# lawfuyang/ToyRenderer

Measured on AMD Instinct MI355X. Metric: Gmeshlets/s culled (whole node), 100M meshlets, higher is better.
Workload: dtype f32

## Files before the change

toyrenderer_amd/csrc/cull_math.hip.h:

```cpp
#pragma once

#include <hip/hip_runtime.h>

#include "ShaderInterop.h"

namespace cm
{

struct F3 { float x, y, z; };

__device__ __forceinline__ float fma_(float a, float b, float c) { return __builtin_fmaf(a, b, c); }
__device__ __forceinline__ float min_(float a, float b) { return __builtin_fminf(a, b); }
__device__ __forceinline__ float max_(float a, float b) { return __builtin_fmaxf(a, b); }
#ifdef TR_EXPERIMENT_FAST_MATH
__device__ __forceinline__ float sqrt_(float a) { return __builtin_amdgcn_sqrtf(a); }
__device__ __forceinline__ float div_(float a, float b) { return a * __builtin_amdgcn_rcpf(b); }
#else
__device__ __forceinline__ float sqrt_(float a) { return __builtin_sqrtf(a); }
__device__ __forceinline__ float div_(float a, float b) { return a / b; }
#endif
__device__ __forceinline__ float clamp_(float x, float lo, float hi) { return min_(max_(x, lo), hi); }

typedef unsigned long long lmask;
__device__ __forceinline__ lmask mLt(float a, float b) { lmask m; asm("v_cmp_lt_f32_e64 %0, %1, %2" : "=s"(m) : "v"(a), "v"(b)); return m; }
// ... 222 lines not shown

__device__ __forceinline__ bool occlusionResolve(const OccSample& o, uint32_t row0, uint32_t row1)
{
    float d00 = texelLo(row0), d10 = texelLo(row1);
    float d01 = o.pair ? texelHi(row0) : d00, d11 = o.pair ? texelHi(row1) : d10;
    float depth = min_(min_(min_(d00, d01), d10), d11);
    return o.accept | (o.depthSphere >= depth);
}

struct HzbQuad
{
    const _Float16* base;
    uint32_t total;
    uint32_t offset[16];
};
__device__ __forceinline__ uint32_t quadIndex(uint32_t offset, uint32_t blockRowStride , uint32_t X, uint32_t Y)
{
    return offset + (__umul24(Y >> 3, blockRowStride) + ((Y << 3) & 56u)) + __umul24(X >> 3, 56u) + X;
}

struct OccQuad
{
    lmask accept;
    lmask slow;
    float depthSphere;
    uint32_t iq;
};

__device__ __forceinline__ bool occlusionVisible(F3 c, float r, float nearPlane, float P00, float P11, const Hzb& h)
{
    if ((c.z - nearPlane) < r) return true;
    OccSample o = occlusionPrepare(c, r, nearPlane, P00, P11, h, h.mipOffset);
    return occlusionResolve(o, loadTexelPair(h.base, o.i0), loadTexelPair(h.base, o.i1));
}

__device__ __forceinline__ float u8Unorm(uint32_t x)
{
    const float r = 0x1.010102p-8f;
    float xf = (float)x;
    float q = xf * r;
    float rem = fma_(-q, 255.0f, xf);
// ... 334 lines not shown
{
    OccQuad o;
    o.accept = mLt(c.z - nearPlane, r);
    const v2f P = { P00, P11 };
    const v2f lo = occClampUv(q.mn, P), hi = occClampUv(q.mx, P);
    const v2f wh = (hi - lo) * v2f{ (float)h.width, (float)h.height };
    const float m = max_(max_(wh.x, wh.y), 1.0f);
    int e = __builtin_amdgcn_frexp_expf(m);
    e = e < (int)h.mips ? e : (int)h.mips;
    e = e > 1 ? e : 1;
    const uint4 tab = mipTab[e];
    const v2f f = fma2(lo + hi, v2f{ __uint_as_float(tab.z), __uint_as_float(tab.w) }, splat2(-0.5f));
    const float flx = __builtin_floorf(f.x), fly = __builtin_floorf(f.y);
    const int x0 = (int)flx, y0 = (int)fly;
    o.iq = min(quadIndex(tab.x, tab.y, (uint32_t)(x0 + 1), (uint32_t)(y0 + 1)), quadTotal - 1u);
    const lmask zx = mNotGt(f.x, flx), zy = mNotGt(f.y, fly);
    o.slow = 0ull;
    if (__builtin_expect((zx | zy) != 0ull, 0)) {
        const int mw = (int)(2.0f * __uint_as_float(tab.z)), mh = (int)(2.0f * __uint_as_float(tab.w));
        const bool bx = !(f.x > flx), by = !(f.y > fly);
        o.slow = __builtin_amdgcn_ballot_w64((bx & (x0 >= 0) & (x0 + 1 < mw)) | (by & (y0 >= 0) & (y0 + 1 < mh)));
    }
    o.depthSphere = q.depthSphere;
    return o;
}

template <bool CONE>
__device__ __forceinline__ void stepDeferred(F3 c, float r, uint32_t packed, const M33P& adj, float nearPlane, const ProjBands& bands, const float* coneTab,
                                             StepQuot& o, lmask& sureOcc, lmask& sureCone)
{
// ... 39 lines not shown
    OccQuad o;
    o.accept = mLt(c.z - nearPlane, r);
    const v2f P = { P00, P11 };
    const v2f lo = occClampUv(mn, P), hi = occClampUv(mx, P);
    const v2f wh = (hi - lo) * v2f{ (float)h.width, (float)h.height };
    const float m = max_(max_(wh.x, wh.y), b.mFloor);
    int e = __builtin_amdgcn_frexp_expf(m);
    e = e < (int)h.mips ? e : (int)h.mips;
    e = e > 1 ? e : 1;
    const uint4 tab = mipTab[e];
    const v2f half = { __uint_as_float(tab.z), __uint_as_float(tab.w) };
    const v2f f = fma2(lo + hi, half, splat2(-0.5f));
    const v2f fl = { __builtin_floorf(f.x), __builtin_floorf(f.y) };
    const int x0 = (int)fl.x, y0 = (int)fl.y;
    o.iq = min(quadIndex(tab.x, tab.y, (uint32_t)(x0 + 1), (uint32_t)(y0 + 1)), quadTotal - 1u);
    const v2f t = f - (fl + splat2(0.5f));
    const v2f cap = fma2(half, -b.K, splat2(0.5f));
    const uint2 band = mipBand[e];
    const uint32_t mb = __float_as_uint(m) + band.x;
    sure &= mAbsLe(t.x, cap.x) & mAbsLe(t.y, cap.y) & mGeU(mb & 0x7FFFFFu, band.y);
    o.slow = 0ull;
    o.depthSphere = depthSphere;
    return o;
}

__device__ __forceinline__ OccSample occTailTexel(const StepQuot& q, F3 c, float r, float nearPlane, float P00, float P11, const Hzb& h, const uint32_t* mipOff)
{
    OccSample o;
    o.accept = (c.z - nearPlane) < r;
    const v2f P = { P00, P11 };
// ... 57 lines not shown
```

toyrenderer_amd/csrc/hzb_quad.hip.h:

```cpp
#pragma once

#include <hip/hip_runtime.h>
#include <cstring>

#include "cull_math.hip.h"
#include "trhip_internal.h"

namespace trhip
{

struct QuadArgs
{
    const _Float16* base;
    _Float16* out;
    uint32_t width, height, mips, total;
    uint32_t mipOffset[16];
    uint32_t quadOffset[16];
    uint32_t blocksPerRow[16];
    uint32_t stripsPerRow[16];
    uint32_t firstStrip[17];
};

constexpr uint32_t kQuadStripBlocks = 32;
constexpr uint32_t kQuadStripCols = kQuadStripBlocks * 8;

__device__ __forceinline__ void hzbQuadStrip(const QuadArgs& a, uint32_t strip_, float (*s_t)[kQuadStripCols + 1], uint32_t tid = threadIdx.x, bool valid = true)
{
    if (!valid) { __syncthreads(); return; }
    uint32_t k = 0;
    for (uint32_t m = 1; m < a.mips; ++m) k += strip_ >= a.firstStrip[m] ? 1u : 0u;
    const uint32_t mw = (a.width >> k) ? (a.width >> k) : 1u, mh = (a.height >> k) ? (a.height >> k) : 1u;
    const uint32_t strip = strip_ - a.firstStrip[k];
    const uint32_t brow = strip / a.stripsPerRow[k], seg = strip - brow * a.stripsPerRow[k];
    const uint32_t X0 = seg * kQuadStripCols, Y0 = brow * 8u;
    const _Float16* __restrict__ t = a.base + a.mipOffset[k];
    {
        const int tx = min(max((int)(X0 + tid) - 1, 0), (int)mw - 1);
        float v[9];
#pragma unroll
        for (uint32_t r = 0; r < 9; ++r) {
            const int ty = min(max((int)(Y0 + r) - 1, 0), (int)mh - 1);
            v[r] = (float)t[(uint32_t)ty * mw + (uint32_t)tx];
        }
// ... 25 lines not shown
    QuadArgs a;
    memset(&a, 0, sizeof a);
    a.base = (const _Float16*)tex->ptr;
    a.out = (_Float16*)tex->quad.ptr;
    a.width = tex->width; a.height = tex->height; a.mips = tex->mips; a.total = tex->quadTotal;
    uint32_t strips = 0;
    for (uint32_t i = 0; i < tex->mips; ++i) {
        a.mipOffset[i] = (uint32_t)(tex->mipOffset[i] / 2);
        a.quadOffset[i] = tex->quadOffset[i];
        a.blocksPerRow[i] = (tex->mipW(i) >> 3) + 1u;
        a.stripsPerRow[i] = (a.blocksPerRow[i] + kQuadStripBlocks - 1u) / kQuadStripBlocks;
        a.firstStrip[i] = strips;
        strips += a.stripsPerRow[i] * ((tex->mipH(i) >> 3) + 1u);
    }
    a.firstStrip[tex->mips] = strips;
    return a;
}

}
```

toyrenderer_amd/csrc/k_basepass_as.hip:

```cpp
#include <algorithm>
#include <cstdlib>
#include <string>
#include <type_traits>

#if defined(TR_STAMPS) || defined(TR_COUNT_SLOW) || defined(TR_COUNT_PATHS)
__device__ unsigned long long g_stampSums[8];
#define g_pathCount (g_stampSums + 4)
#endif
#include <atomic>
#include <memory>
#include <mutex>
#include <unordered_map>

#include "cull_math.hip.h"
#include "instance_cache.hip.h"
#include "meshlet_exact.hip.h"
#include "trhip_internal.h"

using namespace interop;

namespace
{

constexpr uint32_t kBlock = 256;
constexpr uint32_t kWaves = kBlock / 64;
constexpr uint32_t kBatch = 64;
constexpr uint32_t kSteps = kBatch / 2;
#ifndef TR_RING_SLOTS
#define TR_RING_SLOTS 2
// ... 118 lines not shown
#endif
#if TR_LK_POLICY_ID == 0
#define TR_LK_POLICY ""
#elif TR_LK_POLICY_ID == 1
#define TR_LK_POLICY " sc0"
#elif TR_LK_POLICY_ID == 2
#define TR_LK_POLICY " sc1"
#elif TR_LK_POLICY_ID == 3
#define TR_LK_POLICY " sc0 sc1"
#elif TR_LK_POLICY_ID == 4
#define TR_LK_POLICY " nt"
#else
#define TR_LK_POLICY " sc1 nt"
#endif
#ifndef TR_CULL_WAVES_PER_EU
#define TR_CULL_WAVES_PER_EU 5
#endif
template <bool FRUSTUM, bool OCCLUSION, bool CONE, bool TABLE>
__global__ __launch_bounds__(kCullBlock, TR_CULL_WAVES_PER_EU) void meshletCullKernel(MeshletCullArgs a)
{
#ifdef TR_STAMPS
    unsigned long long stampSum[8] = {0, 0, 0, 0, 0, 0, 0, 0};
    unsigned long long stampLast = __builtin_amdgcn_s_memtime();
    __builtin_amdgcn_s_waitcnt(0xC07F);
#endif
    __shared__ RecordInfo s_recAll[kCullWaves][kCullBatch + 2 * kRingSlots];
    __shared__ uint32_t s_gIdxAll[kCullWaves][kCullBatch];
    __shared__ uint32_t s_quadOff[16];
    __shared__ uint4 s_mipTab[17];
    __shared__ float s_coneTab[cm::kConeTabEntries];
    constexpr bool kDeferred = OCCLUSION && TABLE;
    __shared__ uint2 s_mipBand[kDeferred ? 17 : 1];
    __shared__ uint32_t s_defAll[kCullWaves][kDeferred ? kDefStage * kDefWords : 1u];
    __shared__ __attribute__((aligned(8))) uint32_t s_maskAll[kCullWaves][kCullBatch + 2];
    __shared__ __attribute__((aligned(16))) char s_ring[kCullWaves][kRingSlots][kSlotBytes];

    const uint32_t G = groupCount(a);
    const uint32_t tid = threadIdx.x, lane = tid & 63u, wave = tid >> 6;
    const uint32_t half = lane >> 5, sub = lane & 31u;
    if (a.listGroups && blockIdx.x == 0 && tid == 0) a.listGroups[0] = G;
    const cm::M43 V = cm::loadM43(a.k.m_WorldToView);
    const cm::M43P VP = cm::packM43(V);
    const cm::M33P VR = cm::rot(VP);
    const float coneSlack = cm::coneSlackFactor(V);
    if (!TABLE && G <= gridDim.x * (2u * kCullWaves) * a.shortPassRounds) {
        for (uint32_t g = (blockIdx.x * kCullWaves + wave) * 2u + half; g < G; g += gridDim.x * kCullWaves * 2u) {
            const bool vis = exactMeshletVisible<FRUSTUM, OCCLUSION, CONE>(a, VP, VR, g, sub);
            const unsigned long long b = __ballot(vis);
            if (sub == 0) a.visMask[g] = (uint32_t)(half ? b >> 32 : b);
        }
        return;
    }
    RecordInfo* s_rec = s_recAll[wave];
    uint32_t* s_gIdx = s_gIdxAll[wave];

    if (tid < 16) s_quadOff[tid] = a.hzb.mipOffset[tid];
    if (TABLE && tid >= 1 && tid <= 16) {
        const uint32_t mip = tid - 1u < a.hzb.mips ? tid - 1u : 0u;
        const uint32_t mw = (a.hzb.width >> mip) ? (a.hzb.width >> mip) : 1u, mh = (a.hzb.height >> mip) ? (a.hzb.height >> mip) : 1u;
        s_mipTab[tid] = make_uint4(a.quad.offset[mip], ((mw >> 3) + 1u) * 64u, __float_as_uint(0.5f * (float)mw), __float_as_uint(0.5f * (float)mh));
    }
    if (kDeferred && tid >= 1 && tid <= 16) { const uint32_t d = cm::projMipDelta(a.bands, tid); s_mipBand[tid] = make_uint2(d, 2u * d); }
    const bool nearInRange = a.k.m_NearPlane >= 0x1p-20f && a.k.m_NearPlane <= 0x1p20f;
    if (CONE) for (uint32_t i = tid; i < cm::kConeTabEntries; i += kCullBlock) s_coneTab[i] = cm::coneTableEntry(i);
    if (lane < 2 * kRingSlots) { s_recAll[wave][kCullBatch + lane].first = 0; s_recAll[wave][kCullBatch + lane].lastOff = 0; }
    uint32_t* s_def = s_defAll[wave];
    uint32_t* s_mask = s_maskAll[wave];
    __syncthreads();

    const bool usePerm = a.permHeader != nullptr && a.permHeader[0] == 1u && a.permHeader[1] == G;
#ifndef TR_TEAM_ALL
    const uint32_t teamWaves = kCullWaves, waveInTeam = wave, team = blockIdx.x, teams = gridDim.x;
#else
    const uint32_t teamWaves = gridDim.x * kCullWaves, waveInTeam = blockIdx.x * kCullWaves + wave, team = 0u, teams = 1u;
#endif
    const uint32_t superSize = teamWaves * kCullBatch;
    const uint32_t numSuper = (G + superSize - 1) / superSize;
// ... 250 lines not shown
                cm::lmask sureOcc, sureCone;
                cm::stepDeferred<CONE>(cv, rad, cone, adjugateOf(ri), a.k.m_NearPlane, a.bands, s_coneTab, q, sureOcc, sureCone);
                cm::lmask coneUnsure = 0ull;
                if (CONE) {
                    const cm::lmask back = cm::coneBackSure(q, cv, rad, VR, coneSlack, sureCone);
                    coneUnsure = vis & ~sureCone;
                    vis &= ~back;
                }
                cm::lmask unsure = coneUnsure;
                TR_STAMP(3);
                const cm::OccQuad oq = cm::occTailQuadFiltered(q.mn, q.mx, q.depthSphere, cv, rad, a.k.m_NearPlane, a.k.m_P00, a.k.m_P11, a.hzb,
                                                                s_mipTab, s_mipBand, a.quad.total, a.bands, sureOcc);
                if (!nearInRange) sureOcc = 0ull;
                accept = oq.accept; depthSphere = oq.depthSphere;
                unsure |= vis & ~oq.accept & ~sureOcc;
                const uint16_t* entry = reinterpret_cast<const uint16_t*>(a.quad.base) + oq.iq;
#ifdef TR_NO_LOOKUP
                issueLookup(lk0[kSlot], lk1[kSlot], a.quad.base, a.quad.base, 0ull);
                asm volatile("" :: "v"(entry));
#else
                issueLookup(lk0[kSlot], lk1[kSlot], entry, entry, vis & ~oq.accept);
#endif
                if (__builtin_expect(unsure != 0ull, 0)) {
                    const uint32_t n = (uint32_t)__builtin_popcountll(unsure);
                    if (stCount + n > kDefStage) {
                        batchExact = true;
                    } else {
                        const uint32_t at = stCount + __builtin_amdgcn_mbcnt_hi((uint32_t)(unsure >> 32), __builtin_amdgcn_mbcnt_lo((uint32_t)unsure, 0u));
                        if ((unsure >> lane) & 1ull) {
                            uint32_t* d = s_def + at * kDefWords;
                            d[0] = (s_gIdx[r] << 5) | sub;
                            d[1] = CONE && ((coneUnsure >> lane) & 1ull) ? kDefFromRecord : __float_as_uint(cv.x);
                            d[2] = __float_as_uint(cv.y); d[3] = __float_as_uint(cv.z); d[4] = __float_as_uint(rad);
                        }
                        stCount += n;
                    }
// ... 720 lines not shown
        memset(&a.hzb, 0, sizeof a.hzb);
        if (occlusion) {
            TRHIP_REQUIRE(hzb, "%s: occlusion culling enabled but no HZB texture bound at t8", ctx.shaderName);
            TRHIP_REQUIRE(hzb->format == TRHIP_FORMAT_R16_FLOAT, "%s: HZB is not R16_FLOAT", ctx.shaderName);
            TRHIP_REQUIRE(hzb->width == k->m_HZBDimensions.x && hzb->height == k->m_HZBDimensions.y,
                          "%s: m_HZBDimensions %ux%u does not match the HZB texture %ux%u", ctx.shaderName,
                          k->m_HZBDimensions.x, k->m_HZBDimensions.y, hzb->width, hzb->height);
            a.hzb.base = (const _Float16*)hzb->ptr;
            a.hzb.width = hzb->width; a.hzb.height = hzb->height; a.hzb.mips = hzb->mips;
            for (uint32_t m = 0; m < hzb->mips; ++m) a.hzb.mipOffset[m] = (uint32_t)(hzb->mipOffset[m] / 2);
            if (useTable) {
                rc = trhip::hzbQuadEnsure(hzb);
                if (rc != TRHIP_OK) return rc;
                a.quad.base = (const _Float16*)hzb->quad.ptr;
                a.quad.total = hzb->quadTotal;
                for (uint32_t m = 0; m < hzb->mips; ++m) a.quad.offset[m] = hzb->quadOffset[m];
            }
        }
    }
    if (rc != TRHIP_OK) return rc;
    a.meshlets = (const MeshletData*)meshlets->ptr;
    TRHIP_REQUIRE(meshlets->byteSize >= sizeof(MeshletData), "%s: empty meshlet buffer", ctx.shaderName);
    rc = meshlets->cullStream.allocate(meshlets->dev, meshletStreamBytes(meshlets->byteSize / sizeof(MeshletData)));
    if (rc != TRHIP_OK) return rc;
    a.stream = meshletStreamLayout(meshlets->cullStream.ptr, meshlets->byteSize / sizeof(MeshletData));
    a.records = (const MeshletAmplificationData*)records->ptr;
    a.dispatchArgs = (const uint32_t*)((const char*)ctx.argsBuffer->ptr + ctx.argsOffset);
    a.argsWords = (ctx.argsBuffer->byteSize - ctx.argsOffset) >= 16 ? 4u : 3u;
    const uint64_t cap = records->byteSize / sizeof(MeshletAmplificationData);
    a.recordCapacity = cap > 0xFFFFFFFFull ? 0xFFFFFFFFu : (uint32_t)cap;
// ... 29 lines not shown
    uint32_t grid = ctx.computeUnits() * blocksPerCU;
    const uint32_t needBlocks = (a.recordCapacity + kCullBatch * kCullWaves - 1) / (kCullBatch * kCullWaves);
    if (grid > needBlocks) grid = needBlocks;
    if (grid == 0) grid = 1;
    rc = visMask->listCount.allocate(visMask->dev, 256);
    if (rc != TRHIP_OK) return rc;
    a.listGroups = (uint32_t*)visMask->listCount.ptr;
    ctx.cl->use(a.listGroups, ctx.cl->ops.size(), true);
    if (useTable) a.bands = cm::projBands(k->m_P00, k->m_P11, hzb->width, hzb->height);
    static const bool noShortPass = getenv("TRHIP_NO_SHORT_PASS") != nullptr;
    a.shortPassRounds = noShortPass ? 0u : kShortPassRounds;
    const uint32_t flags = k->m_CullingFlags & 7u;
    trhip_texture_t* quadOwner = useTable ? hzb : nullptr;
    const bool table = useTable;
    if (quadOwner) ctx.cl->use(quadOwner->quad.ptr, ctx.cl->ops.size(), false);
    ctx.emit("cull", [a, grid, flags, quadOwner, table, instances, meshData, meshlets](hipStream_t s) {
        if ((const void*)a.meshlets != meshlets->ptr)
            return trhip::fail(TRHIP_ERR_STATE, "basepass_AS_Main: the meshlet buffer was bound to other memory after this command list was recorded: record it again");
        {
            int crc = trhip::instanceCacheLaunchBuild(instances, meshData, s);
            if (crc != TRHIP_OK) return crc;
            crc = meshletStreamLaunchBuild(meshlets, s);
            if (crc != TRHIP_OK) return crc;
        }
        if (quadOwner) {
            int brc = trhip::hzbQuadLaunchBuild(quadOwner, s);
            if (brc != TRHIP_OK) return brc;
        }
        switch (flags) {
        case 0: launchCull<false, false, false>(a, grid, table, s); break;
// ... 157 lines not shown
```

toyrenderer_amd/csrc/k_gpuculling.hip:

```cpp
#include "cull_math.hip.h"
#include "hzb_quad.hip.h"
#include "instance_cache.hip.h"
#include "trhip_internal.h"

using namespace interop;

namespace
{

constexpr uint32_t kBlock = 256;
constexpr uint32_t kWordSubmit = 1u << 30;
constexpr uint32_t kWordLate = 1u << 31;
constexpr uint32_t kGroupMask = (1u << 27) - 1u;

struct InstanceCullArgs
{
    GPUCullingPassConstants k;
    const BasePassInstanceConstants* instances;
    const uint32_t* ids;
    const MeshData* meshData;
    cm::Hzb hzb;
    MeshletAmplificationData* records;
    uint32_t* dispatchArgs;
    uint32_t* lateCount;
// ... 347 lines not shown
                a.lateArgsOut[2] = 1;
            }
        }
        a.permHeader[0] = (n >= kMinBinnedEntries && baseX == 0 && X < a.maxGroups && X <= a.permCapacity) ? 1u : 0u;
        a.permHeader[1] = X;
    }
}

constexpr uint32_t kEmitStripsPerGroup = kBigThreads / 256u;
template <int LATE>
__global__ __launch_bounds__(kBigThreads) void instanceEmitKernel(InstanceCullArgs a, trhip::QuadArgs q, uint32_t stripBegin)
{
    if (!LATE && blockIdx.x >= a.numBlocks) {
        __shared__ float s_t[kEmitStripsPerGroup][9][trhip::kQuadStripCols + 1];
        const uint32_t strip = stripBegin + (blockIdx.x - a.numBlocks) * kEmitStripsPerGroup + (threadIdx.x >> 8);
        trhip::hzbQuadStrip(q, strip, s_t[threadIdx.x >> 8], threadIdx.x & 255u, strip < q.firstStrip[q.mips]);
        return;
    }
    __shared__ uint32_t s_cursor[kNumTiles];
    __shared__ uint32_t s_wave[kBigWaves];
    const uint32_t n = threadCount<LATE>(a);
    if (blockIdx.x >= activeBigBlocks<LATE>(a, n)) return;
    const uint32_t tid = threadIdx.x, lane = tid & 63u, wave = tid >> 6;
    const bool binned = n >= kMinBinnedEntries;
    if (binned) {
        uint32_t carry = 0;
        for (uint32_t base = 0; base < kNumTiles; base += kBigThreads) {
            const bool inRange = base + tid < kNumTiles;
            const uint32_t tot = inRange ? a.tileTotal[base + tid] : 0u;
            const uint32_t inc = waveInclusiveScan(tot, lane);
            if (lane == 63) s_wave[wave] = inc;
// ... 204 lines not shown
                  "%s: m_HZBDimensions %ux%u does not match HZB texture %ux%u", ctx.shaderName, dims.x, dims.y, tex->width, tex->height);
    out->base = (const _Float16*)tex->ptr;
    out->width = tex->width; out->height = tex->height; out->mips = tex->mips;
    for (uint32_t k = 0; k < tex->mips; ++k) out->mipOffset[k] = (uint32_t)(tex->mipOffset[k] / 2);
    return TRHIP_OK;
}

std::function<int(hipStream_t)> fusedEarlyLaunch(const InstanceCullArgs& a, trhip_texture_t* quadOwner)
{
    return [a, quadOwner](hipStream_t s) {
        trhip::QuadArgs q;
        memset(&q, 0, sizeof q);
        uint32_t strips = 0;
        if (quadOwner && !quadOwner->quad.current({ quadOwner->version })) {
            q = trhip::quadArgs(quadOwner);
            strips = q.firstStrip[q.mips];
            quadOwner->quad.markBuilt({ quadOwner->version });
        }
        TRHIP_LAUNCH(instanceFusedKernel<0>, dim3(a.numBlocks + strips), dim3(kBlock), 0, s, a, q);
        return trhip::launchStatus("instanceFusedKernel"); };
}

inline uint32_t quadScanStrips(uint32_t all)
{
    static const uint32_t pct = [] { const char* e = getenv("TRHIP_QUAD_SCAN_PERCENT"); const int v = e ? atoi(e) : 50; return (uint32_t)(v < 0 ? 0 : v > 100 ? 100 : v); }();
    return (uint32_t)((uint64_t)all * pct / 100u);
}

std::function<int(hipStream_t)> scanEarlyLaunch(const InstanceCullArgs& a, trhip_texture_t* quadOwner, std::shared_ptr<QuadShare> share)
{
    return [a, quadOwner, share](hipStream_t s) {
        trhip::QuadArgs q;
        memset(&q, 0, sizeof q);
        uint32_t extra = 0, stripEnd = 0;
        if (share) share->stale = false;
        if (quadOwner && !quadOwner->quad.current({ quadOwner->version })) {
            q = trhip::quadArgs(quadOwner);
            stripEnd = share ? quadScanStrips(q.firstStrip[q.mips]) : q.firstStrip[q.mips];
            extra = (stripEnd + kScanStripsPerGroup - 1u) / kScanStripsPerGroup;
            quadOwner->quad.markBuilt({ quadOwner->version });
            if (share) share->stale = true;
        }
        TRHIP_LAUNCH(instanceScanKernel<0>, dim3(1 + kScanTileGroups + extra), dim3(kScanThreads), 0, s, a, q, stripEnd);
        return trhip::launchStatus("instanceScanKernel"); };
}

template <int LATE>
int recordGPUCulling(trhip::DispatchCtx& ctx)
{
    const GPUCullingPassConstants* k = (const GPUCullingPassConstants*)ctx.constants(0, sizeof(GPUCullingPassConstants));
    TRHIP_REQUIRE(k, "%s: constant buffer b0 (GPUCullingPassConstants, 180 bytes) missing", ctx.shaderName);
    trhip_buffer_t* instances = ctx.buffer(TRHIP_BIND_STRUCTURED_SRV, 0);
    trhip_buffer_t* ids = ctx.buffer(TRHIP_BIND_STRUCTURED_SRV, 1);
    trhip_buffer_t* meshData = ctx.buffer(TRHIP_BIND_STRUCTURED_SRV, 2);
    trhip_texture_t* hzb = ctx.texture(TRHIP_BIND_TEXTURE_SRV, 3);
// ... 72 lines not shown
    if (wantTable) {
        rc = trhip::hzbQuadEnsure(hzb);
        if (rc != TRHIP_OK) return rc;
    }

    if (fusedPath) {
        const size_t words = (size_t)a.numBlocks * kFusedStatusStride * 2 + 4;
        uint32_t* mem = (uint32_t*)ctx.scratch(words * 4);
        TRHIP_REQUIRE(mem, "%s: scratch allocation failed", ctx.shaderName);
        rc = ctx.cl->recordClearWords(mem, words, 0, true);
        if (rc != TRHIP_OK) return rc;
        a.fusedStatus = (unsigned long long*)mem;
        a.fusedTicket = mem + (size_t)a.numBlocks * kFusedStatusStride * 2;
        trhip_texture_t* quadOwner = wantTable ? hzb : nullptr;
        if (quadOwner) ctx.cl->use(quadOwner->quad.ptr, ctx.cl->ops.size(), true);
        if (LATE) ctx.emit("fused", [a](hipStream_t s) {
            trhip::QuadArgs q;
            memset(&q, 0, sizeof q);
            TRHIP_LAUNCH(instanceFusedKernel<LATE>, dim3(a.numBlocks), dim3(kBlock), 0, s, a, q);
            return trhip::launchStatus("instanceFusedKernel"); });
        else ctx.emit("fused", fusedEarlyLaunch(a, quadOwner));
        if (!LATE && occlusion) ctx.cl->peephole = { ctx.cl->ops.size() - 1, "gpuculling_early", std::make_shared<EarlyCullNote>(EarlyCullNote{ a, ctx.cl->ops.size() - 1, true, quadOwner }) };
        return TRHIP_OK;
    }

    ctx.emit("classify", [a](hipStream_t s) {
        TRHIP_LAUNCH(instanceClassifyKernel<LATE>, dim3(a.numBlocks), dim3(kBigThreads), 0, s, a);
        return trhip::launchStatus("instanceClassifyKernel"); });
    trhip_texture_t* quadOwner = wantTable ? hzb : nullptr;
    std::shared_ptr<QuadShare> share = quadOwner ? std::make_shared<QuadShare>() : nullptr;
    if (quadOwner) ctx.cl->use(quadOwner->quad.ptr, ctx.cl->ops.size(), true);
    if (LATE) ctx.emit("scan", [a](hipStream_t s) {
        trhip::QuadArgs q;
        memset(&q, 0, sizeof q);
        TRHIP_LAUNCH(instanceScanKernel<LATE>, dim3(1 + kScanTileGroups), dim3(kScanThreads), 0, s, a, q, 0u);
        return trhip::launchStatus("instanceScanKernel"); });
    else ctx.emit("scan", scanEarlyLaunch(a, quadOwner, share));
    const size_t scanOp = ctx.cl->ops.size() - 1;
    if (quadOwner) ctx.cl->use(quadOwner->quad.ptr, ctx.cl->ops.size(), true);
    ctx.emit("emit", [a, quadOwner, share](hipStream_t s) {
        trhip::QuadArgs q;
        memset(&q, 0, sizeof q);
        uint32_t extra = 0, stripBegin = 0;
        if (!LATE && quadOwner && share && share->stale) {
            q = trhip::quadArgs(quadOwner);
            stripBegin = quadScanStrips(q.firstStrip[q.mips]);
            extra = (q.firstStrip[q.mips] - stripBegin + kEmitStripsPerGroup - 1u) / kEmitStripsPerGroup;
        }
        TRHIP_LAUNCH(instanceEmitKernel<LATE>, dim3(a.numBlocks + extra), dim3(kBigThreads), 0, s, a, q, stripBegin);
        return trhip::launchStatus("instanceEmitKernel"); });
    if (!LATE && occlusion) ctx.cl->peephole = { ctx.cl->ops.size() - 1, "gpuculling_early", std::make_shared<EarlyCullNote>(EarlyCullNote{ a, scanOp, false, quadOwner, share }) };
    return TRHIP_OK;
}

int recordBuildLateArgs(trhip::DispatchCtx& ctx)
{
    trhip_buffer_t* count = ctx.buffer(TRHIP_BIND_STRUCTURED_SRV, 0);
    trhip_buffer_t* args = ctx.buffer(TRHIP_BIND_STRUCTURED_UAV, 0);
    TRHIP_REQUIRE(count && args, "%s: needs SRV t0 (late count) and UAV u0 (indirect args)", ctx.shaderName);
    TRHIP_REQUIRE(count->byteSize >= 4 && args->byteSize >= 12, "%s: buffers too small", ctx.shaderName);
    TRHIP_REQUIRE(!ctx.indirect && ctx.gx == 1 && ctx.gy == 1 && ctx.gz == 1, "%s: dispatched as 1x1x1", ctx.shaderName);
    const uint32_t* c = (const uint32_t*)count->ptr;
// ... 60 lines not shown
```

toyrenderer_amd/csrc/k_hzb.hip:

```cpp
#include "cull_math.hip.h"
#include "hzb_quad.hip.h"
#include "trhip_internal.h"

using namespace interop;

namespace
{

template <bool MAX>
__global__ __launch_bounds__(256) void minMaxDownsampleKernel(const float* __restrict__ depth, uint32_t W, uint32_t H,
                                                              _Float16* __restrict__ out, uint32_t ow, uint32_t oh)
{
    const uint32_t x = blockIdx.x * 32 + (threadIdx.x & 31), y = blockIdx.y * 8 + (threadIdx.x >> 5);
    if (x >= ow || y >= oh) return;
    const float u = ((float)x + 0.5f) / (float)ow, v = ((float)y + 0.5f) / (float)oh;
    const float fx = cm::fma_(u, (float)W, -0.5f), fy = cm::fma_(v, (float)H, -0.5f);
    int x0 = (int)__builtin_floorf(fx), y0 = (int)__builtin_floorf(fy);
    int x1 = min(max(x0 + 1, 0), (int)W - 1), y1 = min(max(y0 + 1, 0), (int)H - 1);
    x0 = min(max(x0, 0), (int)W - 1);
    y0 = min(max(y0, 0), (int)H - 1);
    const float a = depth[(uint64_t)y0 * W + x0], b = depth[(uint64_t)y0 * W + x1];
    const float c = depth[(uint64_t)y1 * W + x0], d = depth[(uint64_t)y1 * W + x1];
    const float r = MAX ? cm::max_(cm::max_(a, b), cm::max_(c, d))
                        : cm::min_(cm::min_(a, b), cm::min_(c, d));
// ... 288 lines not shown
}

namespace trhip
{

int hzbQuadEnsure(trhip_texture_t* tex)
{
    TRHIP_REQUIRE(tex && tex->ptr && tex->format == TRHIP_FORMAT_R16_FLOAT && tex->mips <= 16, "footprint-min table: needs a bound R16_FLOAT texture");
    uint64_t total = 0;
    for (uint32_t k = 0; k < tex->mips; ++k) {
        tex->quadOffset[k] = (uint32_t)total;
        total += (uint64_t)((tex->mipW(k) >> 3) + 1) * ((tex->mipH(k) >> 3) + 1) * 64u;
    }
    TRHIP_REQUIRE(total < (1ull << 31), "footprint-min table: HZB %ux%u too large", tex->width, tex->height);
    tex->quadTotal = (uint32_t)total;
    return tex->quad.allocate(tex->dev, total * 2);
}

int hzbQuadLaunchBuild(trhip_texture_t* tex, hipStream_t s)
{
    const Stamp from = { tex->version };
    if (tex->quad.current(from)) return TRHIP_OK;
    const QuadArgs a = quadArgs(tex);
    TRHIP_LAUNCH(hzbQuadBuildKernel, dim3(a.firstStrip[a.mips]), dim3(256), 0, s, a);
    tex->quad.markBuilt(from);
    return launchStatus("hzbQuadBuildKernel");
}

}

namespace
{

trhip::ShaderRegistrar r0("minmaxdownsample_CS_Main", recordMinMaxDownsample, 0);
trhip::ShaderRegistrar r1("ffx_spd_downsample_pass_CS FFX_SPD_OPTION_DOWNSAMPLE_FILTER=1", recordSPD, 1);
trhip::ShaderRegistrar r2("ffx_spd_downsample_pass_CS FFX_SPD_OPTION_DOWNSAMPLE_FILTER=2", recordSPD, 2);

}
```

toyrenderer_amd/csrc/meshlet_exact.hip.h:

```cpp
#pragma once

#include <hip/hip_runtime.h>

#include "ShaderInterop.h"
#include "cull_math.hip.h"
#include "instance_cache.hip.h"

using namespace interop;

struct MeshletCullStream
{
    const float4* sphere;
    const uint32_t* cone;
};

struct MeshletCullArgs
{
    BasePassConstants k;
    const MeshletData* meshlets;
    MeshletCullStream stream;
    const MeshletAmplificationData* records;
    cm::Hzb hzb;
    cm::HzbQuad quad;
    const uint32_t* dispatchArgs;
    uint32_t argsWords;
    uint32_t recordCapacity;
    uint64_t numMeshlets;
    uint32_t* visMask;
    uint32_t* visibleList; uint32_t listCapacity;
    uint32_t* drawArgs;
    uint32_t* batchSum;
    uint32_t* superSum;
    uint32_t maxBatches;
    const uint32_t* permHeader;
    const uint4* perm;
    InstanceCullCache cache;
    uint32_t numInstances;
    uint32_t* listGroups;
// ... 48 lines not shown
```

toyrenderer_amd/csrc/trhip_core.cpp:

```cpp
#include "trhip_internal.h"
#include "r11g11b10.hip.h"

#include <chrono>
#include <cmath>
#include <cstdlib>

#include <algorithm>
#include <memory>

namespace trhip
{

static thread_local char tl_error[1024] = "";

int fail(int code, const char* fmt, ...)
{
    va_list ap;
    va_start(ap, fmt);
    vsnprintf(tl_error, sizeof tl_error, fmt, ap);
    va_end(ap);
    return code;
}

int hipfail(hipError_t e, const char* what)
// ... 482 lines not shown
    if (t->heap) trhip_heap_release(t->heap);
    heapRetain(heap);
    t->heap = heap;
    t->ptr = (char*)heap->base + offset;
    t->version.fetch_add(1);
    return TRHIP_OK;
}

void trhip_texture_retain(trhip_texture t) { if (t) t->rc.fetch_add(1); }

void trhip_texture_release(trhip_texture t)
{
    if (!t) return;
    if (t->rc.fetch_sub(1) == 1) {
        if (t->owns && t->ptr) { (void)hipSetDevice(t->dev->index); (void)hipFree(t->ptr); }
        trhip::freeDerived(t->dev, { &t->quad });
        if (t->heap) trhip_heap_release(t->heap);
        delete t;
    }
}

void* trhip_texture_device_ptr(trhip_texture t) { return t ? t->ptr : nullptr; }
uint64_t trhip_texture_size(trhip_texture t) { return t ? t->totalBytes : 0; }

int trhip_texture_mip_info(trhip_texture t, uint32_t mip, uint32_t* w, uint32_t* h, uint64_t* off)
{
    if (!t || mip >= t->mips) return fail(TRHIP_ERR_INVALID, "mip_info: bad texture/mip");
    if (w) *w = t->mipW(mip);
    if (h) *h = t->mipH(mip);
    if (off) *off = t->mipOffset[mip];
    return TRHIP_OK;
// ... 632 lines not shown
```

toyrenderer_amd/csrc/trhip_internal.h:

```cpp
#pragma once

#include <hip/hip_runtime.h>

#include <atomic>
#include <cstdarg>
#include <cstdint>
#include <cstdio>
#include <cstdlib>
#include <cstring>
#include <functional>
#include <map>
#include <memory>
#include <mutex>
#include <string>
#include <unordered_map>
#include <vector>

#include <hip/hip_ext.h>

#include "../../include/trhip.h"
#include "ShaderInterop.h"

namespace trhip
{
// ... 106 lines not shown
struct trhip_texture_t
{
    trhip_device_t* dev = nullptr;
    uint32_t width = 0, height = 0, mips = 0, format = 0;
    uint32_t texelBytes = 0;
    bool isUAV = false, isVirtual = false;
    std::string name;
    uint64_t mipOffset[16] = {};
    uint64_t totalBytes = 0;
    void* ptr = nullptr;
    bool owns = false;
    trhip_heap_t* heap = nullptr;
    trhip::DerivedData quad;
    uint32_t quadOffset[16] = {};
    uint32_t quadTotal = 0;
    std::atomic<uint64_t> version{1};
    std::atomic<int> rc{1};

    uint32_t mipW(uint32_t k) const { return (width >> k) ? (width >> k) : 1u; }
    uint32_t mipH(uint32_t k) const { return (height >> k) ? (height >> k) : 1u; }
    void* mipPtr(uint32_t k) const { return (char*)ptr + mipOffset[k]; }
};

struct trhip_timer_t
{
    trhip_device_t* dev = nullptr;
    hipEvent_t e0 = nullptr, e1 = nullptr;
    bool began = false, ended = false;
};

// ... 92 lines not shown
    bool indirect; trhip_buffer_t* argsBuffer; uint32_t argsOffset;
    uint32_t gx, gy, gz;

    trhip_buffer_t* buffer(uint32_t type, uint32_t slot) const;
    trhip_texture_t* texture(uint32_t type, uint32_t slot, uint32_t* baseMip = nullptr) const;
    const void* constants(uint32_t slot, size_t bytes) const;
    uint32_t computeUnits() const { return cl->dev->computeUnits; }
    void* scratch(size_t bytes) const { return cl->scratchAlloc(bytes); }
    void* scratchSide(size_t bytes) const { return cl->dev->sideStream ? cl->scratchAllocSide(bytes) : cl->scratchAlloc(bytes); }
    void emit(const char* kernelName, std::function<int(hipStream_t)> fn) const;
    void emitSide(const char* kernelName, std::function<int(hipStream_t)> fn, std::initializer_list<Op::Access> touched) const;
};

int hzbQuadEnsure(trhip_texture_t* tex);
int hzbQuadLaunchBuild(trhip_texture_t* tex, hipStream_t s);

int instanceCacheEnsure(trhip_buffer_t* instances);
int instanceCacheLaunchBuild(trhip_buffer_t* instances, trhip_buffer_t* meshData, hipStream_t s);

inline uint32_t tableMinGroups()
{
    static const uint32_t v = [] { const char* e = getenv("TRHIP_TABLE_MIN_GROUPS"); return e ? (uint32_t)strtoul(e, nullptr, 0) : (1u << 17); }();
    return v;
}

uint32_t statsCSThreads(const char* shaderName);
int statsLaunchAdd(unsigned long long* counter, uint64_t value, hipStream_t s);
int statsEmitIndirectCS(trhip_cmdlist_t* cl, trhip_buffer_t* args, uint32_t argsOffset, uint32_t threads);
int statsEmitAS(const DispatchCtx& ctx, const ::MeshletCullArgs& a, trhip_buffer_t* meshlets, trhip_buffer_t* records,
                trhip_buffer_t* instances, trhip_buffer_t* meshData, bool side);
// ... 28 lines not shown
```

Before: 122.7.

## Add coarse 64x64 HZB max grid in LDS to decide occlusion early

Builds a 64x64 coarse grid holding the per-cell max depth over each cell's 2x2-cell neighbourhood across the low mips, as extra strips in the HZB quad build. The cull kernel stages this grid in shared memory and, for meshlets already flagged as sure, accepts them as visible when the sphere depth is at least the coarse value, so their global footprint-table lookup is skipped. This adds a build pass, LDS use and a launch-bounds drop from 5 to 4 waves per EU to cover the extra LDS and registers.

After: 115.8. 5.6% lower.

```diff
diff --git a/toyrenderer_amd/csrc/cull_math.hip.h b/toyrenderer_amd/csrc/cull_math.hip.h
--- a/toyrenderer_amd/csrc/cull_math.hip.h
+++ b/toyrenderer_amd/csrc/cull_math.hip.h
@@ -260,6 +260,23 @@
     uint32_t total;
     uint32_t offset[16];
 };
+constexpr uint32_t kCoarseDim = 64, kCoarseNaN = kCoarseDim * kCoarseDim, kCoarseAlloc = kCoarseNaN + 8;
+struct HzbCoarse
+{
+    const _Float16* base;
+    uint32_t sx, sy, K;
+};
+__host__ __device__ inline void coarseLevel(const HzbCoarse& c, uint32_t mip, uint32_t* shx, uint32_t* shy, uint32_t* first)
+{
+    const bool on = c.K != 0xFFFFFFFFu && mip <= c.K;
+    *shx = on ? c.sx - mip : 31u; *shy = on ? c.sy - mip : 31u; *first = on ? 0u : kCoarseNaN;
+}
+__device__ __forceinline__ uint32_t coarseIndex(int x0, int y0, uint32_t shx, uint32_t shy, uint32_t first)
+{
+    const uint32_t cx = (uint32_t)max(x0, 0) >> shx, cy = (uint32_t)max(y0, 0) >> shy;
+    return min(first + cy * kCoarseDim + cx, kCoarseNaN);
+}
+
 __device__ __forceinline__ uint32_t quadIndex(uint32_t offset, uint32_t blockRowStride , uint32_t X, uint32_t Y)
 {
     return offset + (__umul24(Y >> 3, blockRowStride) + ((Y << 3) & 56u)) + __umul24(X >> 3, 56u) + X;
@@ -271,6 +288,7 @@
     lmask slow;
     float depthSphere;
     uint32_t iq;
+    int x0, y0, e;
 };
 
 __device__ __forceinline__ bool occlusionVisible(F3 c, float r, float nearPlane, float P00, float P11, const Hzb& h)
@@ -635,6 +653,7 @@
     const float flx = __builtin_floorf(f.x), fly = __builtin_floorf(f.y);
     const int x0 = (int)flx, y0 = (int)fly;
     o.iq = min(quadIndex(tab.x, tab.y, (uint32_t)(x0 + 1), (uint32_t)(y0 + 1)), quadTotal - 1u);
+    o.x0 = x0; o.y0 = y0; o.e = e;
     const lmask zx = mNotGt(f.x, flx), zy = mNotGt(f.y, fly);
     o.slow = 0ull;
     if (__builtin_expect((zx | zy) != 0ull, 0)) {
@@ -704,6 +723,7 @@
     const v2f fl = { __builtin_floorf(f.x), __builtin_floorf(f.y) };
     const int x0 = (int)fl.x, y0 = (int)fl.y;
     o.iq = min(quadIndex(tab.x, tab.y, (uint32_t)(x0 + 1), (uint32_t)(y0 + 1)), quadTotal - 1u);
+    o.x0 = x0; o.y0 = y0; o.e = e;
     const v2f t = f - (fl + splat2(0.5f));
     const v2f cap = fma2(half, -b.K, splat2(0.5f));
     const uint2 band = mipBand[e];
diff --git a/toyrenderer_amd/csrc/hzb_quad.hip.h b/toyrenderer_amd/csrc/hzb_quad.hip.h
--- a/toyrenderer_amd/csrc/hzb_quad.hip.h
+++ b/toyrenderer_amd/csrc/hzb_quad.hip.h
@@ -19,7 +19,65 @@
     uint32_t blocksPerRow[16];
     uint32_t stripsPerRow[16];
     uint32_t firstStrip[17];
+    _Float16* coarse;
+    uint32_t coarseSx, coarseSy, coarseK, coarseGx, coarseGy;
+    uint32_t strips;
 };
+
+inline void coarseShape(uint32_t w, uint32_t h, uint32_t mips, uint32_t* gx, uint32_t* gy, uint32_t* sx, uint32_t* sy, uint32_t* K)
+{
+    *gx = *gy = *sx = *sy = 0u; *K = 0xFFFFFFFFu;
+    if (!w || !h || !mips || (w & (w - 1u)) || (h & (h - 1u))) return;
+    *gx = w < cm::kCoarseDim ? w : cm::kCoarseDim; *gy = h < cm::kCoarseDim ? h : cm::kCoarseDim;
+    for (uint32_t v = w / *gx; v > 1u; v >>= 1) ++*sx;
+    for (uint32_t v = h / *gy; v > 1u; v >>= 1) ++*sy;
+    *K = *sx < *sy ? *sx : *sy;
+    if (*K > mips - 1u) *K = mips - 1u;
+}
+
+constexpr uint32_t kCoarseStrips = cm::kCoarseNaN / 4u;
+#ifndef TR_COARSE_MIP0_ONLY
+#define TR_COARSE_MIP0_ONLY 0
+#endif
+__device__ __forceinline__ uint32_t coarseKey(uint32_t b) { return b ^ ((b & 0x8000u) ? 0xFFFFu : 0x8000u); }
+__device__ __forceinline__ void hzbCoarseStrip(const QuadArgs& a, uint32_t cs, uint32_t tid)
+{
+    const uint32_t lane = tid & 63u, entry = cs * 4u + (tid >> 6);
+    const uint32_t cx = entry & (cm::kCoarseDim - 1u), cy = entry / cm::kCoarseDim;
+    const bool on = a.coarseK != 0xFFFFFFFFu && cx < a.coarseGx && cy < a.coarseGy;
+    const uint16_t* __restrict__ base = reinterpret_cast<const uint16_t*>(a.base);
+    uint32_t key = 0u;
+    bool nan = false;
+    auto take = [&](uint32_t b) { nan |= (b & 0x7FFFu) > 0x7C00u; key = max(key, coarseKey(b)); };
+    const uint32_t lastMip = !on ? 0u : TR_COARSE_MIP0_ONLY ? 1u : a.coarseK + 1u;
+    for (uint32_t k = 0; k < lastMip; ++k) {
+        const uint32_t lw = a.coarseSx - k, lh = a.coarseSy - k;
+        const uint32_t mw = a.coarseGx << lw, mh = a.coarseGy << lh;
+        const uint32_t x0 = cx << lw, y0 = cy << lh;
+        const uint32_t rw = min((cx + 2u) << lw, mw) - x0, rh = min((cy + 2u) << lh, mh) - y0;
+        const uint16_t* __restrict__ t = base + a.mipOffset[k] + (uint64_t)y0 * mw + x0;
+        const uint32_t lrw = 31u - (uint32_t)__builtin_clz(rw);
+        if (lw >= 3u && (reinterpret_cast<uintptr_t>(base + a.mipOffset[k]) & 15u) == 0u) {
+            const uint32_t lu = lrw - 3u, n = rh << lu;
+            for (uint32_t i = lane; i < n; i += 64u) {
+                const uint4 v = *reinterpret_cast<const uint4*>(t + (uint64_t)(i >> lu) * mw + ((i & ((1u << lu) - 1u)) << 3));
+                take(v.x & 0xFFFFu); take(v.x >> 16); take(v.y & 0xFFFFu); take(v.y >> 16);
+                take(v.z & 0xFFFFu); take(v.z >> 16); take(v.w & 0xFFFFu); take(v.w >> 16);
+            }
+        } else {
+            const uint32_t n = rh << lrw;
+            for (uint32_t i = lane; i < n; i += 64u) take(t[(uint64_t)(i >> lrw) * mw + (i & (rw - 1u))]);
+        }
+    }
+#pragma unroll
+    for (int d = 32; d >= 1; d >>= 1) key = max(key, (uint32_t)__shfl_xor((int)key, d));
+    const bool anyNan = __ballot(nan) != 0ull;
+    if (lane == 0) {
+        const uint32_t bits = !on || anyNan ? 0x7E00u : key ^ ((key & 0x8000u) ? 0x8000u : 0xFFFFu);
+        reinterpret_cast<uint16_t*>(a.coarse)[entry] = (uint16_t)bits;
+    }
+    if (cs == 0u && tid < cm::kCoarseAlloc - cm::kCoarseNaN) reinterpret_cast<uint16_t*>(a.coarse)[cm::kCoarseNaN + tid] = 0x7E00u;
+}
 
 constexpr uint32_t kQuadStripBlocks = 32;
 constexpr uint32_t kQuadStripCols = kQuadStripBlocks * 8;
@@ -27,6 +85,7 @@
 __device__ __forceinline__ void hzbQuadStrip(const QuadArgs& a, uint32_t strip_, float (*s_t)[kQuadStripCols + 1], uint32_t tid = threadIdx.x, bool valid = true)
 {
     if (!valid) { __syncthreads(); return; }
+    if (strip_ >= a.firstStrip[a.mips]) { hzbCoarseStrip(a, strip_ - a.firstStrip[a.mips], tid); __syncthreads(); return; }
     uint32_t k = 0;
     for (uint32_t m = 1; m < a.mips; ++m) k += strip_ >= a.firstStrip[m] ? 1u : 0u;
     const uint32_t mw = (a.width >> k) ? (a.width >> k) : 1u, mh = (a.height >> k) ? (a.height >> k) : 1u;
@@ -82,6 +141,9 @@
         strips += a.stripsPerRow[i] * ((tex->mipH(i) >> 3) + 1u);
     }
     a.firstStrip[tex->mips] = strips;
+    a.coarse = (_Float16*)tex->coarse.ptr;
+    coarseShape(tex->width, tex->height, tex->mips, &a.coarseGx, &a.coarseGy, &a.coarseSx, &a.coarseSy, &a.coarseK);
+    a.strips = strips + kCoarseStrips;
     return a;
 }
 
diff --git a/toyrenderer_amd/csrc/k_basepass_as.hip b/toyrenderer_amd/csrc/k_basepass_as.hip
--- a/toyrenderer_amd/csrc/k_basepass_as.hip
+++ b/toyrenderer_amd/csrc/k_basepass_as.hip
@@ -13,6 +13,7 @@
 #include <unordered_map>
 
 #include "cull_math.hip.h"
+#include "hzb_quad.hip.h"
 #include "instance_cache.hip.h"
 #include "meshlet_exact.hip.h"
 #include "trhip_internal.h"
@@ -161,7 +162,7 @@
 #define TR_LK_POLICY " sc1 nt"
 #endif
 #ifndef TR_CULL_WAVES_PER_EU
-#define TR_CULL_WAVES_PER_EU 5
+#define TR_CULL_WAVES_PER_EU 4
 #endif
 template <bool FRUSTUM, bool OCCLUSION, bool CONE, bool TABLE>
 __global__ __launch_bounds__(kCullBlock, TR_CULL_WAVES_PER_EU) void meshletCullKernel(MeshletCullArgs a)
@@ -178,6 +179,8 @@
     __shared__ float s_coneTab[cm::kConeTabEntries];
     constexpr bool kDeferred = OCCLUSION && TABLE;
     __shared__ uint2 s_mipBand[kDeferred ? 17 : 1];
+    __shared__ __attribute__((aligned(16))) uint16_t s_coarse[kDeferred ? cm::kCoarseAlloc : 8u];
+    __shared__ uint4 s_coarseTab[kDeferred ? 17 : 1];
     __shared__ uint32_t s_defAll[kCullWaves][kDeferred ? kDefStage * kDefWords : 1u];
     __shared__ __attribute__((aligned(8))) uint32_t s_maskAll[kCullWaves][kCullBatch + 2];
     __shared__ __attribute__((aligned(16))) char s_ring[kCullWaves][kRingSlots][kSlotBytes];
@@ -208,6 +211,18 @@
         s_mipTab[tid] = make_uint4(a.quad.offset[mip], ((mw >> 3) + 1u) * 64u, __float_as_uint(0.5f * (float)mw), __float_as_uint(0.5f * (float)mh));
     }
     if (kDeferred && tid >= 1 && tid <= 16) { const uint32_t d = cm::projMipDelta(a.bands, tid); s_mipBand[tid] = make_uint2(d, 2u * d); }
+    if (kDeferred) {
+        static_assert(cm::kCoarseNaN * 2u == 2u * 16u * kCullBlock, "coarse grid staging: two 16-byte loads per thread");
+        const uint4* src = reinterpret_cast<const uint4*>(a.coarse.base);
+        uint4* dst = reinterpret_cast<uint4*>(s_coarse);
+        dst[tid] = src[tid]; dst[tid + kCullBlock] = src[tid + kCullBlock];
+        if (tid < cm::kCoarseAlloc - cm::kCoarseNaN) s_coarse[cm::kCoarseNaN + tid] = 0x7E00u;
+        if (tid >= 1 && tid <= 16) {
+            uint32_t shx, shy, first;
+            cm::coarseLevel(a.coarse, tid - 1u, &shx, &shy, &first);
+            s_coarseTab[tid] = make_uint4(shx, shy, first, 0u);
+        }
+    }
     const bool nearInRange = a.k.m_NearPlane >= 0x1p-20f && a.k.m_NearPlane <= 0x1p20f;
     if (CONE) for (uint32_t i = tid; i < cm::kConeTabEntries; i += kCullBlock) s_coneTab[i] = cm::coneTableEntry(i);
     if (lane < 2 * kRingSlots) { s_recAll[wave][kCullBatch + lane].first = 0; s_recAll[wave][kCullBatch + lane].lastOff = 0; }
@@ -488,12 +503,23 @@
                 if (!nearInRange) sureOcc = 0ull;
                 accept = oq.accept; depthSphere = oq.depthSphere;
                 unsure |= vis & ~oq.accept & ~sureOcc;
+#ifndef TR_NO_COARSE
+                {
+                    const uint4 ct = s_coarseTab[oq.e];
+                    const float F = (float)__builtin_bit_cast(_Float16, s_coarse[cm::coarseIndex(oq.x0, oq.y0, ct.x, ct.y, ct.z)]);
+                    const cm::lmask decided = sureOcc & vis & cm::mGe(depthSphere, F);
+#ifdef TR_COUNT_PATHS
+                    if (lane == 0) { atomicAdd(&g_stampSums[6], (unsigned long long)__builtin_popcountll(vis & ~oq.accept)); atomicAdd(&g_stampSums[7], (unsigned long long)__builtin_popcountll(decided & ~oq.accept)); }
+#endif
+                    accept |= decided;
+                }
+#endif
                 const uint16_t* entry = reinterpret_cast<const uint16_t*>(a.quad.base) + oq.iq;
 #ifdef TR_NO_LOOKUP
                 issueLookup(lk0[kSlot], lk1[kSlot], a.quad.base, a.quad.base, 0ull);
                 asm volatile("" :: "v"(entry));
 #else
-                issueLookup(lk0[kSlot], lk1[kSlot], entry, entry, vis & ~oq.accept);
+                issueLookup(lk0[kSlot], lk1[kSlot], entry, entry, vis & ~accept);
 #endif
                 if (__builtin_expect(unsure != 0ull, 0)) {
                     const uint32_t n = (uint32_t)__builtin_popcountll(unsure);
@@ -1244,6 +1270,8 @@
                 if (rc != TRHIP_OK) return rc;
                 a.quad.base = (const _Float16*)hzb->quad.ptr;
                 a.quad.total = hzb->quadTotal;
+                a.coarse.base = (const _Float16*)hzb->coarse.ptr;
+                { uint32_t gx, gy; trhip::coarseShape(hzb->width, hzb->height, hzb->mips, &gx, &gy, &a.coarse.sx, &a.coarse.sy, &a.coarse.K); }
                 for (uint32_t m = 0; m < hzb->mips; ++m) a.quad.offset[m] = hzb->quadOffset[m];
             }
         }
@@ -1303,6 +1331,7 @@
     trhip_texture_t* quadOwner = useTable ? hzb : nullptr;
     const bool table = useTable;
     if (quadOwner) ctx.cl->use(quadOwner->quad.ptr, ctx.cl->ops.size(), false);
+    if (quadOwner) ctx.cl->use(quadOwner->coarse.ptr, ctx.cl->ops.size(), false);
     ctx.emit("cull", [a, grid, flags, quadOwner, table, instances, meshData, meshlets](hipStream_t s) {
         if ((const void*)a.meshlets != meshlets->ptr)
             return trhip::fail(TRHIP_ERR_STATE, "basepass_AS_Main: the meshlet buffer was bound to other memory after this command list was recorded: record it again");
diff --git a/toyrenderer_amd/csrc/k_gpuculling.hip b/toyrenderer_amd/csrc/k_gpuculling.hip
--- a/toyrenderer_amd/csrc/k_gpuculling.hip
+++ b/toyrenderer_amd/csrc/k_gpuculling.hip
@@ -385,7 +385,7 @@
     if (!LATE && blockIdx.x >= a.numBlocks) {
         __shared__ float s_t[kEmitStripsPerGroup][9][trhip::kQuadStripCols + 1];
         const uint32_t strip = stripBegin + (blockIdx.x - a.numBlocks) * kEmitStripsPerGroup + (threadIdx.x >> 8);
-        trhip::hzbQuadStrip(q, strip, s_t[threadIdx.x >> 8], threadIdx.x & 255u, strip < q.firstStrip[q.mips]);
+        trhip::hzbQuadStrip(q, strip, s_t[threadIdx.x >> 8], threadIdx.x & 255u, strip < q.strips);
         return;
     }
     __shared__ uint32_t s_cursor[kNumTiles];
@@ -620,8 +620,8 @@
         uint32_t strips = 0;
         if (quadOwner && !quadOwner->quad.current({ quadOwner->version })) {
             q = trhip::quadArgs(quadOwner);
-            strips = q.firstStrip[q.mips];
-            quadOwner->quad.markBuilt({ quadOwner->version });
+            strips = q.strips;
+            trhip::hzbQuadMarkBuilt(quadOwner);
         }
         TRHIP_LAUNCH(instanceFusedKernel<0>, dim3(a.numBlocks + strips), dim3(kBlock), 0, s, a, q);
         return trhip::launchStatus("instanceFusedKernel"); };
@@ -642,9 +642,9 @@
         if (share) share->stale = false;
         if (quadOwner && !quadOwner->quad.current({ quadOwner->version })) {
             q = trhip::quadArgs(quadOwner);
-            stripEnd = share ? quadScanStrips(q.firstStrip[q.mips]) : q.firstStrip[q.mips];
+            stripEnd = share ? quadScanStrips(q.strips) : q.strips;
             extra = (stripEnd + kScanStripsPerGroup - 1u) / kScanStripsPerGroup;
-            quadOwner->quad.markBuilt({ quadOwner->version });
+            trhip::hzbQuadMarkBuilt(quadOwner);
             if (share) share->stale = true;
         }
         TRHIP_LAUNCH(instanceScanKernel<0>, dim3(1 + kScanTileGroups + extra), dim3(kScanThreads), 0, s, a, q, stripEnd);
@@ -747,6 +747,7 @@
         a.fusedTicket = mem + (size_t)a.numBlocks * kFusedStatusStride * 2;
         trhip_texture_t* quadOwner = wantTable ? hzb : nullptr;
         if (quadOwner) ctx.cl->use(quadOwner->quad.ptr, ctx.cl->ops.size(), true);
+        if (quadOwner) ctx.cl->use(quadOwner->coarse.ptr, ctx.cl->ops.size(), true);
         if (LATE) ctx.emit("fused", [a](hipStream_t s) {
             trhip::QuadArgs q;
             memset(&q, 0, sizeof q);
@@ -763,6 +764,7 @@
     trhip_texture_t* quadOwner = wantTable ? hzb : nullptr;
     std::shared_ptr<QuadShare> share = quadOwner ? std::make_shared<QuadShare>() : nullptr;
     if (quadOwner) ctx.cl->use(quadOwner->quad.ptr, ctx.cl->ops.size(), true);
+    if (quadOwner) ctx.cl->use(quadOwner->coarse.ptr, ctx.cl->ops.size(), true);
     if (LATE) ctx.emit("scan", [a](hipStream_t s) {
         trhip::QuadArgs q;
         memset(&q, 0, sizeof q);
@@ -771,14 +773,15 @@
     else ctx.emit("scan", scanEarlyLaunch(a, quadOwner, share));
     const size_t scanOp = ctx.cl->ops.size() - 1;
     if (quadOwner) ctx.cl->use(quadOwner->quad.ptr, ctx.cl->ops.size(), true);
+    if (quadOwner) ctx.cl->use(quadOwner->coarse.ptr, ctx.cl->ops.size(), true);
     ctx.emit("emit", [a, quadOwner, share](hipStream_t s) {
         trhip::QuadArgs q;
         memset(&q, 0, sizeof q);
         uint32_t extra = 0, stripBegin = 0;
         if (!LATE && quadOwner && share && share->stale) {
             q = trhip::quadArgs(quadOwner);
-            stripBegin = quadScanStrips(q.firstStrip[q.mips]);
-            extra = (q.firstStrip[q.mips] - stripBegin + kEmitStripsPerGroup - 1u) / kEmitStripsPerGroup;
+            stripBegin = quadScanStrips(q.strips);
+            extra = (q.strips - stripBegin + kEmitStripsPerGroup - 1u) / kEmitStripsPerGroup;
         }
         TRHIP_LAUNCH(instanceEmitKernel<LATE>, dim3(a.numBlocks + extra), dim3(kBigThreads), 0, s, a, q, stripBegin);
         return trhip::launchStatus("instanceEmitKernel"); });
diff --git a/toyrenderer_amd/csrc/k_hzb.hip b/toyrenderer_amd/csrc/k_hzb.hip
--- a/toyrenderer_amd/csrc/k_hzb.hip
+++ b/toyrenderer_amd/csrc/k_hzb.hip
@@ -326,16 +326,25 @@
     }
     TRHIP_REQUIRE(total < (1ull << 31), "footprint-min table: HZB %ux%u too large", tex->width, tex->height);
     tex->quadTotal = (uint32_t)total;
-    return tex->quad.allocate(tex->dev, total * 2);
+    int rc = tex->quad.allocate(tex->dev, total * 2);
+    if (rc != TRHIP_OK) return rc;
+    return tex->coarse.allocate(tex->dev, cm::kCoarseAlloc * 2);
+}
+
+void hzbQuadMarkBuilt(trhip_texture_t* tex)
+{
+    const Stamp from = { tex->version };
+    tex->quad.markBuilt(from);
+    tex->coarse.markBuilt(from);
 }
 
 int hzbQuadLaunchBuild(trhip_texture_t* tex, hipStream_t s)
 {
     const Stamp from = { tex->version };
-    if (tex->quad.current(from)) return TRHIP_OK;
+    if (tex->quad.current(from) && tex->coarse.current(from)) return TRHIP_OK;
     const QuadArgs a = quadArgs(tex);
-    TRHIP_LAUNCH(hzbQuadBuildKernel, dim3(a.firstStrip[a.mips]), dim3(256), 0, s, a);
-    tex->quad.markBuilt(from);
+    TRHIP_LAUNCH(hzbQuadBuildKernel, dim3(a.strips), dim3(256), 0, s, a);
+    hzbQuadMarkBuilt(tex);
     return launchStatus("hzbQuadBuildKernel");
 }
 
diff --git a/toyrenderer_amd/csrc/meshlet_exact.hip.h b/toyrenderer_amd/csrc/meshlet_exact.hip.h
--- a/toyrenderer_amd/csrc/meshlet_exact.hip.h
+++ b/toyrenderer_amd/csrc/meshlet_exact.hip.h
@@ -22,6 +22,7 @@
     const MeshletAmplificationData* records;
     cm::Hzb hzb;
     cm::HzbQuad quad;
+    cm::HzbCoarse coarse;
     const uint32_t* dispatchArgs;
     uint32_t argsWords;
     uint32_t recordCapacity;
diff --git a/toyrenderer_amd/csrc/trhip_core.cpp b/toyrenderer_amd/csrc/trhip_core.cpp
--- a/toyrenderer_amd/csrc/trhip_core.cpp
+++ b/toyrenderer_amd/csrc/trhip_core.cpp
@@ -520,7 +520,7 @@
     if (!t) return;
     if (t->rc.fetch_sub(1) == 1) {
         if (t->owns && t->ptr) { (void)hipSetDevice(t->dev->index); (void)hipFree(t->ptr); }
-        trhip::freeDerived(t->dev, { &t->quad });
+        trhip::freeDerived(t->dev, { &t->quad, &t->coarse });
         if (t->heap) trhip_heap_release(t->heap);
         delete t;
     }
diff --git a/toyrenderer_amd/csrc/trhip_internal.h b/toyrenderer_amd/csrc/trhip_internal.h
--- a/toyrenderer_amd/csrc/trhip_internal.h
+++ b/toyrenderer_amd/csrc/trhip_internal.h
@@ -144,6 +144,7 @@
     trhip::DerivedData quad;
     uint32_t quadOffset[16] = {};
     uint32_t quadTotal = 0;
+    trhip::DerivedData coarse;
     std::atomic<uint64_t> version{1};
     std::atomic<int> rc{1};
 
@@ -266,6 +267,7 @@
 
 int hzbQuadEnsure(trhip_texture_t* tex);
 int hzbQuadLaunchBuild(trhip_texture_t* tex, hipStream_t s);
+void hzbQuadMarkBuilt(trhip_texture_t* tex);
 
 int instanceCacheEnsure(trhip_buffer_t* instances);
 int instanceCacheLaunchBuild(trhip_buffer_t* instances, trhip_buffer_t* meshData, hipStream_t s);
```
